# xiezhy6/PASTA-GAN

Measured on AMD Instinct MI355X. Metric: training images/sec at 256x192 (tensor 256x256), batch 16 per GPU, higher is better.
Workload: dtype f32

## Files before the change

### pasta-gan_amd/csrc/conv_igemm.hip

```cpp
#include "conv_launch.h"

namespace pasta {

static void launch_fwd_bf16x6(bool tile128, bool rows, const ConvFwdParams& p, hipStream_t s) {
    const int BM = tile128 ? 128 : 64, BN = tile128 ? 128 : 256;
    ConvFwdParams q = p;
    q.o_tiles = (p.Og + BM - 1) / BM;
    int64_t tiles = 0;
    for (int c = 0; c < p.ncls; c++) {
        const int64_t t = ceil_div64((int64_t)p.N * p.cls[c].P * p.cls[c].Q, BN);
        if (t > tiles) tiles = t;
    }
    tiles *= p.ncls;
    const dim3 grid((unsigned)tiles, q.o_tiles * q.ksplit, p.G);
    if (rows) { if (tile128) tu_fwd_rows_128(q, grid, s); else tu_fwd_rows_64(q, grid, s); }
    else      { if (tile128) tu_fwd_base_128(q, grid, s); else tu_fwd_base_64(q, grid, s); }
}

static void launch_fwd_rows2d(int kernel, const ConvFwdParams& p, hipStream_t s) {
    ConvFwdParams q = p;
    q.rows_y0 = p.tap_dy[0];
    for (int t = 1; t < 9; t++) q.rows_y0 = p.tap_dy[t] < q.rows_y0 ? p.tap_dy[t] : q.rows_y0;
    if (kernel == PASTA_FWD_ROWS2D_WIDE) { if (q.x_pieces) tu_rows2d_wide_pieces(q, s); else tu_rows2d_wide(q, s); }
    else if (kernel == PASTA_FWD_ROWS2D_R4) tu_rows2d_128_r4(q, s);
    else if (kernel == PASTA_FWD_ROWS2D_R2) tu_rows2d_128_r2(q, s);
    else tu_rows2d_64_r8(q, s);
}

static void launch_lattice(const FwdChoice& c, const ConvFwdParams& p, hipStream_t s) {
    if (c.kernel == PASTA_FWD_F32) tu_fwd_f32(c.tile, p, s);
    else if (is_rows2d(c.kernel)) launch_fwd_rows2d(c.kernel, p, s);
    else launch_fwd_bf16x6(c.tile == T128x128, c.kernel == PASTA_FWD_ROWS, p, s);
}

static void set_lattice(ConvFwdParams& p, const TapTable& t) {
    p.ncls = t.ncls;
    for (int c = 0; c < 4; c++) p.cls[c] = {t.cls[c].P, t.cls[c].Q, t.cls[c].oy0, t.cls[c].ox0, t.cls[c].T, t.cls[c].tap0};
    memcpy(p.tap_dy, t.tap_dy, sizeof(p.tap_dy)); memcpy(p.tap_dx, t.tap_dx, sizeof(p.tap_dx)); memcpy(p.tap_slab, t.tap_slab, sizeof(p.tap_slab));
    p.isy = t.isy; p.isx = t.isx; p.osy = t.osy; p.osx = t.osx;
    p.rows = t.rows; p.rows_d0 = t.rows_d0; p.rows_rev = t.rows_rev;
    const TapTable::Lattice& l = t.cls[t.ncls > 0 ? t.ncls - 1 : 0];
    p.P = l.P; p.Q = l.Q; p.oy0 = l.oy0; p.ox0 = l.ox0; p.T = l.T;
}

static float desc_wscale(const pasta_conv_desc* d) { return d->wscale == 0.f ? 1.f : d->wscale; }

static inline int launch_flags_of(const float* iscale, const float* oscale, const pasta_conv_epilogue* ep, const float* wmod_s) {
    return (iscale ? PASTA_PLAN_ISCALE : 0) | (oscale ? PASTA_PLAN_OSCALE : 0) | (ep ? PASTA_PLAN_EPILOGUE : 0) | (wmod_s ? PASTA_PLAN_MODULATED : 0) |
           (ep && ep->noise ? PASTA_PLAN_NOISE : 0);
}

static void launch_transposed_pairs(const pasta_conv_desc* d, const ConvFwdParams& base, FwdTile tile, hipStream_t s, const EdgeWeights& ew) {
    TapTable rem;
    lattice_pair_remainder(d, rem);
    if (rem.ncls) {
        ConvFwdParams q = base;
        set_lattice(q, rem);
        tu_conv_t2_edge(q, ew, s);
    }
    PairLattice pl;
    lattice_pair_main(d, pl);
    ConvFwdParams p = base;
    set_lattice(p, pl.t);
    p.pair_bx = pl.pair_bx;
    for (int i = 0; i < 3; i++) p.pair_off[i] = pl.pair_off[i];
    if (tile == T128x128) tu_fwd_pair_128(p, s); else tu_fwd_pair_64(p, s);
}

static int conv2d_run(const void* x, const float* w, void* y, const float* iscale, const float* oscale,
                      const pasta_conv_epilogue* ep, const pasta_conv_desc* d, void* workspace, int64_t workspace_bytes,
                      void* stream, const float* wmod_s, const float* wmod_d);
static int wgrad_run(const void* xv, const void* dyv, float* dw, const pasta_conv_desc* d, void* workspace, int64_t workspace_bytes, void* stream,
                     const float* mod_s, const float* mod_w, float* ds);

static bool pack_job_of(const pasta_conv_desc* d, void* workspace, PackJob& j) {
    const FwdChoice c = choose_fwd(d, 0);
    FwdWorkspace lay;
    if (c.pieces != NP_F16X3 || c.packed || d->io_dtype != PASTA_F32 || d->x2 || fwd_workspace(d, c.plan, lay)) return false;
    const int Ig = d->C_in / d->groups, Og = d->C_out / d->groups;
    j.rowinv = (float*)workspace + lay.rowinv;
    j.wp = (float*)workspace + lay.pack;
    j.G = d->groups; j.Ig = Ig; j.Og = Og;
    j.Ig_pad = round_up(Ig, fwd_ipad(Ig, c.tile)); j.Og_pad = round_up(Og, fwd_tile_bm(c.tile));
    j.kh = d->kh; j.kw = d->kw; j.transposed = d->transposed; j.flip = d->flip;
    j.wscale = desc_wscale(d);
    j.pack_xcd_rows = (j.Og_pad & 63) == 0 ? 1 : 0;
    return true;
}

}


extern "C" int64_t pasta_conv2d_workspace(const pasta_conv_desc* d) {
    using namespace pasta;
    FwdWorkspace lay;
    if (check_desc(d, "conv2d_workspace") || fwd_workspace(d, plan_fwd(d), lay)) return -1;
    return lay.total_floats * (int64_t)sizeof(float);
}

extern "C" int pasta_conv2d_tile(const pasta_conv_desc* d) {
    using namespace pasta;
    if (check_desc(d, "conv2d_tile")) return -1;
    return (int)plan_fwd(d).tile;
}

extern "C" int pasta_conv2d_plan(const pasta_conv_desc* d, int launch_flags, int* tile, int* ksplit, int* math, int* launches, int* kernel) {
    using namespace pasta;
    if (int e = check_desc(d, "conv2d_plan")) return e;
    const FwdChoice c = choose_fwd(d, launch_flags);
    if (d->io_dtype != PASTA_F32 && !c.pieces && !is_fewch(c.kernel))
        return fail("conv2d: no 16-bit-storage kernel for this shape (fewer than 16 input channels per group, at most 32 "
                    "output channels, or an input scale -- pointwise layers over more than 8192 pixels excepted): convert the tensors to fp32 for this launch");
    if (tile) *tile = (int)c.tile;
    if (ksplit) *ksplit = c.ksplit;
    if (math) *math = c.math;
    if (launches) *launches = c.launches;
    if (kernel) *kernel = c.kernel;
    if (d->x_layout == PASTA_LAYOUT_PIECES16 && !c.pieces_ok)
        return fail("conv2d: x_layout = PASTA_LAYOUT_PIECES16 is served by the 3x3 stride-2 forward kernel (conv2d, pad 0, fp32 y, PASTA_MATH_F16X3, one group, "
                    "C_in a multiple of 8 and >= 16, C_out > 32, output width a power of two >= 16, more than 8192 output pixels, no scale vectors) and by the "
                    "eight-wave 3x3 stride-1 tile kernel (plan kernel 7, no input scale, C_in a multiple of 8) only");
    return 0;
}

extern "C" int pasta_conv2d(const void* x, const float* w, void* y, const float* iscale, const float* oscale,
                            const pasta_conv_desc* d, void* workspace, int64_t workspace_bytes, void* stream) {
    return pasta_conv2d_ex(x, w, y, iscale, oscale, nullptr, d, workspace, workspace_bytes, stream);
}

extern "C" int pasta_conv2d_ex(const void* x, const float* w, void* y, const float* iscale, const float* oscale,
                               const pasta_conv_epilogue* ep, const pasta_conv_desc* d, void* workspace, int64_t workspace_bytes,
                               void* stream) {
    return pasta::conv2d_run(x, w, y, iscale, oscale, ep, d, workspace, workspace_bytes, stream, nullptr, nullptr);
}

extern "C" int pasta_conv2d_modulated(const void* x, const float* w, const float* styles, const float* dcoefs, void* y,
                                      const pasta_conv_epilogue* ep, const pasta_conv_desc* d, void* workspace, int64_t workspace_bytes,
                                      void* stream) {
    using namespace pasta;
    PASTA_CHECK(styles, "conv2d_modulated: null styles");
    return conv2d_run(x, w, y, nullptr, nullptr, ep, d, workspace, workspace_bytes, stream, styles, dcoefs);
}

extern "C" int pasta_conv2d_pack_pair(const float* w, const pasta_conv_desc* da, void* ws_a, int64_t ws_a_bytes, const pasta_conv_desc* db, void* ws_b,
                                      int64_t ws_b_bytes, void* stream, int* packed_mask) {
    using namespace pasta;
    PASTA_CHECK(w && da && db && ws_a && ws_b && packed_mask, "conv2d_pack_pair: null pointer");
    *packed_mask = 0;
    if (int e = check_desc(da, "conv2d_pack_pair")) return e;
    if (int e = check_desc(db, "conv2d_pack_pair")) return e;
    PASTA_CHECK(ws_a_bytes >= pasta_conv2d_workspace(da) && ws_b_bytes >= pasta_conv2d_workspace(db), "conv2d_pack_pair: workspace too small");
    PASTA_CHECK((((uintptr_t)ws_a | (uintptr_t)ws_b) & 15) == 0, "conv2d_pack_pair: workspaces must be 16-byte aligned");
    PackJob a, b;
    if (da->groups != db->groups || !pack_job_of(da, ws_a, a) || !pack_job_of(db, ws_b, b)) return 0;
    tu_pack_weights_f16x3_pair(w, a, b, (hipStream_t)stream);
    *packed_mask = 3;
    return launch_status("conv2d_pack_pair");
}

int pasta::conv2d_run(const void* x, const float* w, void* y, const float* iscale, const float* oscale,
                      const pasta_conv_epilogue* ep, const pasta_conv_desc* d, void* workspace, int64_t workspace_bytes,
                      void* stream, const float* wmod_s, const float* wmod_d) {
    if (int e = check_desc(d, "conv2d")) return e;
    PASTA_CHECK(!ep || (ep->act >= 1 && ep->act <= 3), "conv2d: fused epilogue supports act 1..3 (linear, relu, lrelu), got %d", ep ? ep->act : 0);
    PASTA_CHECK(!ep || !ep->noise || ep->noise_strength, "conv2d: noise without noise_strength");
    PASTA_CHECK(x && w && y, "conv2d: null pointer");
    const FwdChoice ch = choose_fwd(d, launch_flags_of(iscale, oscale, ep, wmod_s));
    FwdWorkspace lay;
    if (int e = fwd_workspace(d, ch.plan, lay)) return e;
    const int64_t need = lay.total_floats * (int64_t)sizeof(float);
    PASTA_CHECK(workspace && workspace_bytes >= need, "conv2d: workspace of %lld bytes needed, %lld given", (long long)need, (long long)workspace_bytes);
    PASTA_CHECK(((uintptr_t)workspace & 15) == 0, "conv2d: workspace must be 16-byte aligned");
    hipStream_t s = (hipStream_t)stream;
    if (is_fewch(ch.kernel)) {
        FewChParams q;
        q.x = x; q.w = w; q.y = y; q.iscale = iscale; q.io = d->io_dtype;
        q.bias = ep ? ep->bias : nullptr; q.res = ep ? ep->res : nullptr; q.y_amax = ep ? ep->y_amax : nullptr;
        q.N = d->N; q.Cin = d->C_in; q.Cout = d->C_out; q.HW = d->H * d->W;
        q.w_io = d->transposed ? 1 : 0;
        q.wscale = desc_wscale(d);
        q.act = ep ? ep->act : 0; q.alpha = ep ? ep->alpha : 0.f; q.gain = ep ? ep->gain : 1.f; q.clamp = ep ? ep->clamp : -1.f;
        tu_conv1x1_fewch(ch.kernel == PASTA_FWD_FEWCIN ? 1 : 2, q, s);
        return launch_status("conv2d");
// ... 259 lines not shown
```

### pasta-gan_amd/csrc/conv_launch.h

```cpp
#pragma once
#include "conv_common.h"

namespace pasta {

void tu_pack_weights_f32(const float* w, float* wp, int G, int Ig, int Og, int Ig_pad, int Og_pad, int kh, int kw, int transposed, int flip,
                         float wscale, const float* mod_s, const float* mod_d, hipStream_t s);
void tu_pack_weights_bf16(const float* w, void* wp, int G, int Ig, int Og, int Ig_pad, int Og_pad, int kh, int kw, int transposed, int flip,
                          float wscale, int f16, const float* mod_s, const float* mod_d, hipStream_t s);
void tu_pack_weights_f16x3(const float* w, void* wp, float* rowinv, int G, int Ig, int Og, int Ig_pad, int Og_pad, int kh, int kw, int transposed,
                           int flip, float wscale, const float* mod_s, const float* mod_d, int pack_xcd_rows, hipStream_t s);
void tu_pack_weights_f16x3_pair(const float* w, const PackJob& a, const PackJob& b, hipStream_t s);
void tu_fwd_f32(FwdTile t, const ConvFwdParams& p, hipStream_t s);

void tu_fwd_base_128(const ConvFwdParams& q, dim3 grid, hipStream_t s);
void tu_fwd_base_64(const ConvFwdParams& q, dim3 grid, hipStream_t s);
void tu_fwd_rows_128(const ConvFwdParams& q, dim3 grid, hipStream_t s);
void tu_fwd_rows_64(const ConvFwdParams& q, dim3 grid, hipStream_t s);
void tu_fwd_pair_128(const ConvFwdParams& p, hipStream_t s);
void tu_fwd_pair_64(const ConvFwdParams& p, hipStream_t s);

void tu_rows2d_wide(const ConvFwdParams& q, hipStream_t s);
void tu_rows2d_wide_pieces(const ConvFwdParams& q, hipStream_t s);
void tu_rows2d_128_r4(const ConvFwdParams& q, hipStream_t s);
void tu_rows2d_128_r2(const ConvFwdParams& q, hipStream_t s);
void tu_rows2d_64_r8(const ConvFwdParams& q, hipStream_t s);

void tu_conv1x1(const ConvFwdParams& p, hipStream_t s);
void tu_conv3x3s2(const ConvFwdParams& p, hipStream_t s);

void tu_conv_t2(const ConvFwdParams& p, hipStream_t s);

void tu_conv1x1_fewch(int kind, const FewChParams& p, hipStream_t s);

void tu_splitk_reduce(const ConvFwdParams& p, hipStream_t s);
void tu_amax_times(const float* parts_in, const float* v, int n, float* parts_out, hipStream_t s);
struct EdgeWeights { const float* w; const float* mod_s; const float* mod_d; float wscale; int flip; };
void tu_conv_t2_edge(const ConvFwdParams& q, const EdgeWeights& ew, hipStream_t s);
void tu_packed_koff(unsigned* koff, int K, int kh, int kw, int flip, int HWp, int Wp, hipStream_t s);
void tu_pad_planes(const float* x, float* xp, int64_t planes, int H, int W, int ph, int pw, hipStream_t s);

int  tu_wgrad_f32(int TR, int TS, int WA, int pipe, int kp, const WgradParams& p, int64_t blocks, size_t lds_bytes, hipStream_t s);
void tu_wgrad_reduce(const float* slab, float* dw, int ksplit, int G, int Ag, int Bg, int Ag_pad, int Bg_pad, int kh, int kw, int flip, float wscale,
                     hipStream_t s);
void tu_wgrad_reduce_modulated(bool mod_a, dim3 grid, const float* slab, const float* sty, const float* w, float* dw, float* dsp, int ksplit, int N,
                               int Ag, int Bg, int Ap, int Bp, int kh, int kw, int flip, float wscale, int wg_rows, hipStream_t s);
void tu_sum_blocks(const float* blocks, float* out, int nblocks, int n, hipStream_t s);
void tu_wgrad_smallcin(const WgradSmallParams& q, int blocks, size_t lds_bytes, hipStream_t s);
void tu_wgrad_smallcin_reduce(const float* slab, float* dw, int ksplit, int Ag, int bprime, int a_pad, int bpad, float wscale, hipStream_t s);
void tu_wgrad1x1_fewcin(int CI, int io, dim3 grid, const void* dy, const void* x, float* slab, int N, int Co, int HW, int64_t quads_per_slice, int a_pad,
                        int bpad, hipStream_t s);

void tu_wgrad3x3(int np, const WgradParams& p, int64_t blocks, hipStream_t s);
void tu_wgrad3x3s2(int np, const WgradParams& p, int64_t blocks, hipStream_t s);
void tu_wgrad1x1(int np, int WA, const WgradParams& p, int64_t blocks, hipStream_t s);

}
```

### pasta-gan_amd/csrc/conv_plan.h

```cpp
#ifndef PASTA_CONV_PLAN_H
#define PASTA_CONV_PLAN_H
#include <stddef.h>
#include <stdlib.h>
#include "../../include/pasta_hip.h"
#include "host_common.h"

namespace pasta {

constexpr int MAX_TAPS = 49;
constexpr int NP_F16X3 = 4;
constexpr int AMAX_PARTS = 256;
constexpr int WS_AMAX_FLOATS = 2 * AMAX_PARTS;

enum FwdTile { T128x128 = 0, T64x256 = 1, T32x256 = 2, T64x64 = 3 };

static inline int fwd_tile_bm(FwdTile t) { return t == T128x128 ? 128 : t == T32x256 ? 32 : 64; }
static inline int fwd_tile_bn(FwdTile t) { return t == T128x128 ? 128 : 256; }

static inline int round_up(int a, int b) { return (a + b - 1) / b * b; }


static inline bool is_rows2d(int k) { return k >= PASTA_FWD_ROWS2D_R4 && k <= PASTA_FWD_ROWS2D_WIDE; }
static inline bool is_fewch(int k) { return k == PASTA_FWD_FEWCIN || k == PASTA_FWD_FEWCOUT; }
static inline bool wgrad_split(int k) { return k == PASTA_WGRAD_3X3 || k == PASTA_WGRAD_3X3S2 || k == PASTA_WGRAD_1X1 || k == PASTA_WGRAD_3X3S2_PIECES; }


static inline int check_desc(const pasta_conv_desc* d, const char* who) {
    PASTA_CHECK(d, "%s: null descriptor", who);
    PASTA_CHECK(d->N >= 1 && d->C_in >= 1 && d->H >= 1 && d->W >= 1 && d->C_out >= 1 && d->OH >= 1 && d->OW >= 1,
                "%s: empty tensor in descriptor", who);
    PASTA_CHECK(d->kh >= 1 && d->kw >= 1 && d->kh * d->kw <= MAX_TAPS, "%s: kernel %dx%d unsupported (max %d taps)", who, d->kh, d->kw, MAX_TAPS);
    PASTA_CHECK(d->stride >= 1 && d->stride <= 4, "%s: stride %d unsupported", who, d->stride);
    PASTA_CHECK(d->pad_h >= 0 && d->pad_w >= 0, "%s: negative padding", who);
    PASTA_CHECK(d->math >= PASTA_MATH_DEFAULT && d->math <= PASTA_MATH_F16X3, "%s: unknown math mode %d", who, d->math);
    PASTA_CHECK(d->io_dtype == PASTA_F32 || d->io_dtype == PASTA_F16 || d->io_dtype == PASTA_BF16, "%s: io_dtype %d is not PASTA_F32 / PASTA_F16 / PASTA_BF16", who, d->io_dtype);
    PASTA_CHECK(d->groups >= 1 && d->C_in % d->groups == 0 && d->C_out % d->groups == 0, "%s: channels not divisible by groups=%d", who, d->groups);
    PASTA_CHECK(d->x_layout == PASTA_LAYOUT_NCHW || d->x_layout == PASTA_LAYOUT_PIECES16, "%s: unknown x_layout %d", who, d->x_layout);
    if (!d->transposed) {
        const int oh = (d->H + 2 * d->pad_h - d->kh) / d->stride + 1, ow = (d->W + 2 * d->pad_w - d->kw) / d->stride + 1;
        PASTA_CHECK(d->H + 2 * d->pad_h >= d->kh && d->W + 2 * d->pad_w >= d->kw && oh == d->OH && ow == d->OW,
                    "%s: conv2d output is %dx%d, descriptor says %dx%d", who, oh, ow, d->OH, d->OW);
    } else {
        const int oh = (d->H - 1) * d->stride - 2 * d->pad_h + d->kh, ow = (d->W - 1) * d->stride - 2 * d->pad_w + d->kw;
        PASTA_CHECK(d->OH >= oh && d->OH < oh + d->stride && d->OW >= ow && d->OW < ow + d->stride,
                    "%s: conv_transpose2d output %dx%d not in [%d,%d)x[%d,%d)", who, d->OH, d->OW, oh, oh + d->stride, ow, ow + d->stride);
    }
    PASTA_CHECK((int64_t)d->N * d->C_in * d->H * d->W <= INT32_MAX && (int64_t)d->N * d->C_out * d->OH * d->OW <= INT32_MAX,
                "%s: tensor too large", who);
    return 0;
}


static inline bool split_arith(const pasta_conv_desc* d) { return d->math != PASTA_MATH_F32 || d->io_dtype != PASTA_F32; }
static inline bool doubled_plane(const pasta_conv_desc* d) { return d->OH >= 2 * d->H && d->OH <= 2 * d->H + 1 && d->OW >= 2 * d->W && d->OW <= 2 * d->W + 1; }
static inline bool doubled_remainder(const pasta_conv_desc* d) { return d->OH > 2 * d->H || d->OW > 2 * d->W; }
static inline bool is_3x3(const pasta_conv_desc* d) { return d->kh == 3 && d->kw == 3; }
static inline bool pads_0_or_1(const pasta_conv_desc* d) { return d->pad_h == d->pad_w && d->pad_h <= 1; }

struct SLDims { int P, Q, LH, LW; };
static inline SLDims sl_dims(const pasta_conv_desc* d) {
    return d->transposed ? SLDims{d->H, d->W, d->OH, d->OW} : SLDims{d->OH, d->OW, d->H, d->W};
}

static inline int math_pieces(int math) { return math == PASTA_MATH_BF16 ? 1 : math == PASTA_MATH_BF16X3 ? 2 : math == PASTA_MATH_BF16X6 ? 3 : NP_F16X3; }
static inline bool fp32_equivalent(int pieces) { return pieces == 3 || pieces == NP_F16X3; }


static inline bool rows_tile_ok(int P, int Q, int BN) {
    const int seg = Q < BN ? Q : BN;
    return Q % 32 == 0 && (seg & (seg - 1)) == 0 && BN % seg == 0 && Q % seg == 0 && ((int64_t)P * Q) % BN == 0;
}

template <int BN, int R>
static inline bool rows2d_tile_ok(int P, int Q) {
    constexpr int SEG = BN / R;
    return P % R == 0 && Q % SEG == 0;
}
static inline int rows2d_rows(int P, int Q) {
    if (rows2d_tile_ok<128, 4>(P, Q)) return 4;
    return rows2d_tile_ok<128, 2>(P, Q) ? 2 : 0;
}
static inline bool rows2d_r8(int P, int Q) { return rows2d_tile_ok<256, 8>(P, Q); }

static inline bool conv3x3s2_shape_ok(int OH, int OW) {
    if (OW < 16 || (OW & (OW - 1))) return false;
    const int seg = OW < 128 ? OW : 128, R = 128 / seg;
    return OH % R == 0;
}

static inline int conv1x1_fewch_kind(const pasta_conv_desc* d, bool has_iscale, bool has_oscale, bool has_noise, bool modulated) {
    if (d->kh != 1 || d->kw != 1 || d->stride != 1 || d->pad_h || d->pad_w || d->groups != 1) return 0;
    if (has_oscale || has_noise || modulated || d->x2 || d->x_layout || d->OH != d->H || d->OW != d->W) return 0;
    const int64_t hw = (int64_t)d->H * d->W;
    if (hw % 4 || (int64_t)d->N * hw <= 8192) return 0;
    if (d->C_in <= 16 && !has_iscale && d->C_out >= 16 && d->C_out <= 512) return 1;
    if (d->C_out <= 16 && d->C_in >= 16 && (int64_t)d->C_in * ((d->C_out + 3) & ~3) * 4 <= 64 * 1024) return 2;
    return 0;
}

static inline int wgrad_mod_rows(int Ap, int Bp, int KK) { return (int64_t)(Bp / 64) * (Ap / 16) * KK >= 512 ? 16 : 4; }

struct WgradChunks { int cw_log2, qblocks, chunks_total; };
static inline WgradChunks wgrad_chunks(int kp, int rows_total, int Q, bool keep_width = false) {
    WgradChunks c;
    int cw = kp, lg = kp == 32 ? 5 : 4;
    while (cw > 1 && cw / 2 >= Q && !keep_width) { cw /= 2; lg--; }
    const int chh = kp / cw;
    c.cw_log2 = lg;
    c.qblocks = (Q + cw - 1) / cw;
    c.chunks_total = ((rows_total + chh - 1) / chh) * c.qblocks;
    return c;
}


static inline int fwd_ipad(int Ig, FwdTile t) { return (Ig <= 4 && t == T64x256) ? 4 : Ig <= 8 ? 8 : 16; }

static inline int64_t fwd_lattice_pixels(const pasta_conv_desc* d) {
    if (!d->transposed) return (int64_t)d->N * d->OH * d->OW;
    return (int64_t)d->N * ((d->OH + d->stride - 1) / d->stride) * ((d->OW + d->stride - 1) / d->stride);
}

struct FwdPlan { FwdTile tile; int ksplit; int bf16x6; int packed; };

static inline bool isc_in_staging(const pasta_conv_desc* d) { return d->io_dtype == PASTA_F32 && fp32_equivalent(math_pieces(d->math)); }

static inline FwdPlan plan_fwd(const pasta_conv_desc* d) {
    const int Og = d->C_out / d->groups, Ig = d->C_in / d->groups;
    const int64_t npix = fwd_lattice_pixels(d);
    const bool sb = split_arith(d) && Ig >= 16 && (int64_t)d->N * d->C_in * d->H * d->W < (1ll << 30);
    const bool few = !d->transposed && d->groups == 1 && Ig < 16 && Og > 32 && npix > 8192 && d->io_dtype == PASTA_F32 &&
                     d->math != PASTA_MATH_F32 && fp32_equivalent(math_pieces(d->math)) && Ig * d->kh * d->kw >= 64 && Ig * d->kh * d->kw <= 1024 &&
                     (int64_t)d->N * d->C_in * (d->H + 2 * d->pad_h) * (d->W + 2 * d->pad_w) < (1ll << 28);
    FwdPlan f;
    f.packed = few;
    if (Og <= 32 && !(sb && Og > 16 && npix > 8192)) f.tile = T32x256;
    else if (npix <= 8192) f.tile = (sb && Og > 64) ? T128x128 : T64x64;
    else if (Og <= 64) f.tile = T64x256;
    else f.tile = T128x128;
    f.bf16x6 = (sb || few) && (f.tile == T128x128 || f.tile == T64x256);
    f.packed = f.packed && f.bf16x6;
    f.ksplit = 1;
    if (npix <= 8192 && f.tile != T32x256) {
        const int bm = fwd_tile_bm(f.tile), bn = f.tile == T64x64 ? 64 : 128;
        int64_t blocks = ceil_div64(npix, bn) * ((Og + bm - 1) / bm) * d->groups;
        const int taps = d->transposed ? 1 : d->kh * d->kw;
        if (d->transposed && f.bf16x6 && d->stride == 2) blocks *= 4;
        const int64_t k_total = (int64_t)taps * round_up(Ig, 16);
        int64_t ks = (f.tile == T64x64 ? 768 : 512) / (blocks > 0 ? blocks : 1);
        if (ks > k_total / 64) ks = k_total / 64;
        if (ks > 32) ks = 32;
        f.ksplit = ks < 2 ? 1 : (int)ks;
    }
    return f;
}

static inline bool merged_classes(const pasta_conv_desc* d, bool bf16x6) {
    return d->transposed && bf16x6 && d->stride == 2 && d->OH >= 2 && d->OW >= 2;
}

static inline bool t2_3x3_doubled(const pasta_conv_desc* d, int ksplit) {
    return d->transposed && d->stride == 2 && is_3x3(d) && d->io_dtype == PASTA_F32 && ksplit == 1 && doubled_plane(d);
}

static inline bool pair_launch_ok(const pasta_conv_desc* d, int pieces, int ksplit, FwdTile tile, bool pair_small) {
    if (!t2_3x3_doubled(d, ksplit) || !pads_0_or_1(d) || !fp32_equivalent(pieces)) return false;
    if (tile != T128x128 && tile != T64x256) return false;
    if (doubled_remainder(d) && (int64_t)d->H * d->W < 128 * 128 && !pair_small) return false;
    return rows_tile_ok(d->H, d->W, fwd_tile_bn(tile));
}

static inline bool t2_shape_ok(const pasta_conv_desc* d, int pieces, int ksplit) {
    if (!t2_3x3_doubled(d, ksplit) || d->pad_h != 0 || d->pad_w != 0) return false;
    if (pieces != NP_F16X3 || d->x2 || d->x_layout) return false;
    return d->C_in / d->groups >= 16 && ((d->H % 8 == 0 && d->W % 32 == 0) || (d->H % 16 == 0 && d->W % 16 == 0));
}

enum TransposedLaunch { TL_NONE, TL_ONEPASS, TL_PAIR, TL_MERGED, TL_PER_CLASS };

struct FwdChoice {
    int kernel;
    FwdPlan plan;
    FwdTile tile;
    int ksplit;
    int pieces;
    int math;
    int launches;
    TransposedLaunch tl;
    bool packed;
    bool pieces_ok;
};

static inline FwdChoice choose_fwd(const pasta_conv_desc* d, int launch_flags) {
    static const int rows2d_mode = getenv("PASTA_ROWS2D") ? atoi(getenv("PASTA_ROWS2D")) : 8;
    static const bool pair_small = getenv("PASTA_T2_PAIR") && getenv("PASTA_T2_PAIR")[0] == '2';
    const bool iscale = launch_flags & PASTA_PLAN_ISCALE, oscale = launch_flags & PASTA_PLAN_OSCALE;
    const bool modulated = launch_flags & PASTA_PLAN_MODULATED, noise = launch_flags & PASTA_PLAN_NOISE;
    const FwdPlan f = plan_fwd(d);
    const int np = math_pieces(d->math);
    const bool f32 = d->io_dtype == PASTA_F32;
    FwdChoice c;
    c.plan = f;
    c.tile = f.tile;
    c.tl = TL_NONE;
    c.packed = false;
    c.pieces = 0;
    c.pieces_ok = false;
    if (const int few = conv1x1_fewch_kind(d, iscale, oscale, noise, modulated)) {
        c.kernel = few == 1 ? PASTA_FWD_FEWCIN : PASTA_FWD_FEWCOUT; c.ksplit = 1; c.math = PASTA_MATH_F32; c.launches = 1;
        return c;
    }
    c.ksplit = f.ksplit;
    const bool sb = f.bf16x6 && (!iscale || isc_in_staging(d)) && !(f.packed && (iscale || modulated));
    c.packed = sb && f.packed;
    c.pieces = !sb ? 0 : !f32 ? 1 : np;
    c.math = !sb ? PASTA_MATH_F32 : !f32 ? PASTA_MATH_BF16 : d->math == PASTA_MATH_BF16X3 ? PASTA_MATH_BF16X3 : d->math == PASTA_MATH_BF16 ? PASTA_MATH_BF16 :
             d->math == PASTA_MATH_BF16X6 ? PASTA_MATH_BF16X6 : PASTA_MATH_F16X3;
    const bool f16x3 = sb && f32 && np == NP_F16X3;
    const int bn1 = (d->C_out / d->groups) <= 64 ? 256 : 128;
    const bool c1x1 = f16x3 && d->groups == 1 && d->kh == 1 && d->kw == 1 && d->stride == 1 && !d->pad_h && !d->pad_w && !iscale && !oscale && !noise &&
                      c.ksplit == 1 && !c.packed && d->C_in >= 16 && d->C_out > 32 && d->OH == d->H && d->OW == d->W && ((int64_t)d->H * d->W) % bn1 == 0;
    const bool s2_fits = f16x3 && !d->transposed && d->groups == 1 && is_3x3(d) && d->stride == 2 && pads_0_or_1(d) &&
                         !iscale && !oscale && c.ksplit == 1 && !c.packed && d->C_in >= 16 && d->C_out > 32 && conv3x3s2_shape_ok(d->OH, d->OW);
    const bool s2 = s2_fits && !noise;
    const bool t2 = sb && t2_shape_ok(d, np, c.ksplit) && !(launch_flags & ~(PASTA_PLAN_ISCALE | PASTA_PLAN_MODULATED));
    const bool pair = !t2 && sb && !(launch_flags & ~PASTA_PLAN_MODULATED) && pair_launch_ok(d, np, c.ksplit, c.tile, pair_small);
    const bool rows = sb && d->stride == 1 && d->kw == 3 && rows_tile_ok(d->OH, d->OW, fwd_tile_bn(c.tile));
    const bool plain6 = sb && d->stride == 1 && is_3x3(d) && rows2d_mode != 0;
    const int rows2d = plain6 && c.tile == T128x128 ? rows2d_rows(d->OH, d->OW) : 0;
    const bool rows2d_256 = plain6 && c.tile == T64x256 && rows2d_r8(d->OH, d->OW);
    const bool wide = rows2d && rows2d_mode == 8 && (!iscale || np == NP_F16X3) && fp32_equivalent(np) && f32 && rows2d_r8(d->OH, d->OW);
    c.kernel = !sb ? PASTA_FWD_F32 : c1x1 ? PASTA_FWD_1X1 : s2 ? PASTA_FWD_3X3S2 : c.packed ? PASTA_FWD_PACKED_K : t2 ? PASTA_FWD_T2 : pair ? PASTA_FWD_PAIR :
               wide ? PASTA_FWD_ROWS2D_WIDE : rows2d ? (rows2d == 4 ? PASTA_FWD_ROWS2D_R4 : PASTA_FWD_ROWS2D_R2) : rows2d_256 ? PASTA_FWD_ROWS2D_R8 :
               rows ? PASTA_FWD_ROWS : PASTA_FWD_BASE;
    if (d->transposed)
        c.tl = t2 ? TL_ONEPASS : pair ? TL_PAIR : merged_classes(d, sb) ? TL_MERGED : TL_PER_CLASS;
    c.launches = c.tl == TL_PAIR ? 1 + (doubled_remainder(d) ? 1 : 0) : c.tl != TL_PER_CLASS ? 1 :
                 (d->stride < d->OH ? d->stride : d->OH) * (d->stride < d->OW ? d->stride : d->OW);
    c.pieces_ok = f16x3 && d->groups == 1 && !(launch_flags & (PASTA_PLAN_ISCALE | PASTA_PLAN_MODULATED)) && d->C_in >= 16 && (d->C_in & 7) == 0 && !d->x2 &&
                  (wide || (s2_fits && d->pad_h == 0));
    return c;
}

struct FwdWorkspace { int64_t rowinv, pack, partial, koff, extra, total_floats; };

static inline int fwd_workspace(const pasta_conv_desc* d, const FwdPlan& f, FwdWorkspace& ws) {
    const int Ig = d->C_in / d->groups, Og_pad = round_up(d->C_out / d->groups, fwd_tile_bm(f.tile));
    int64_t pack = ((int64_t)d->groups * d->kh * d->kw * round_up(Ig, fwd_ipad(Ig, f.tile)) * Og_pad * 3 + 1) / 2;
    const int64_t partial = f.ksplit > 1 ? (int64_t)f.ksplit * d->N * d->C_out * d->OH * d->OW : 0;
    int64_t koff = 0, extra = 0;
    if (f.packed) {
        koff = round_up(Ig * d->kh * d->kw, 16);
        const int64_t pk = (koff * Og_pad * 3 + 1) / 2;
        pack = pack > pk ? pack : pk;
        if (d->pad_h || d->pad_w) extra = (int64_t)d->N * d->C_in * (d->H + 2 * d->pad_h) * (d->W + 2 * d->pad_w);
    }
    const bool t2 = t2_shape_ok(d, math_pieces(d->math), f.ksplit);
    if (t2) { koff = 0; extra = (int64_t)d->N * d->C_in * d->H; }
    PASTA_CHECK(!(f.packed || t2) || partial == 0, "conv2d: the packed-K table and the one-pass kernel's column exist without K slices only");
    ws.rowinv = WS_AMAX_FLOATS;
    ws.pack = ws.rowinv + (int64_t)d->groups * Og_pad;
    ws.partial = ws.pack + round_up((int)pack, 4);
    ws.koff = ws.partial + partial;
    ws.extra = ws.koff + koff;
    ws.total_floats = ws.koff + round_up((int)(koff + extra), 4);
    return 0;
}


struct WgradPlan {
    int TR, TS, WA, WB, pipe, npos, kp, bf16x6, tgr, tgs, a_tiles, b_tiles, cw_log2, qblocks, chunks_total, ksplit, rows_total;
    int64_t slab_floats; size_t lds_bytes;
};

static inline bool wgrad_3x3s1_same(const pasta_conv_desc* d, const SLDims& t) {
    return split_arith(d) && is_3x3(d) && d->stride == 1 && d->pad_h == 1 && d->pad_w == 1 && t.LH == t.P && t.LW == t.Q;
}

static inline bool wgrad_wide16(const pasta_conv_desc* d) {
    const SLDims t = sl_dims(d);
    return wgrad_3x3s1_same(d, t) && t.Q == 16 && !d->x_layout;
}

static inline WgradPlan plan_wgrad(int N, int P, int Q, int G, int Ag, int Bg, int kh, int kw, int st, int ks_multiple = 1, bool wide16 = false) {
    WgradPlan w;
    w.bf16x6 = 0;
    if (kh == 3 && kw == 3) { w.TR = 3; w.TS = 3; }
    else if (kw == 7) { w.TR = 1; w.TS = 7; }
    else if (kw == 4) { w.TR = 1; w.TS = 4; }
    else { w.TR = 1; w.TS = 1; }
    w.WA = w.WB = (w.TR * w.TS == 1 && Ag > 64 && Bg > 64) ? 2 : 1;
    const int BA = 64 * w.WA, BB = 64 * w.WB;
    w.tgr = (kh + w.TR - 1) / w.TR; w.tgs = (kw + w.TS - 1) / w.TS;
    w.a_tiles = (Ag + BA - 1) / BA; w.b_tiles = (Bg + BB - 1) / BB;
    int kp = 32;
    w.rows_total = N * P;
    for (;;) {
        const WgradChunks c = wgrad_chunks(kp, w.rows_total, Q, wide16);
        const int cw = 1 << c.cw_log2, chh = kp >> c.cw_log2;
        const int lwid = (cw - 1) * st + w.TS;
        w.cw_log2 = c.cw_log2; w.qblocks = c.qblocks; w.chunks_total = c.chunks_total;
        w.kp = kp; w.npos = chh * w.TR * lwid;
        if (w.npos <= 128 || kp == 16) break;
        kp = 16;
    }
    const int cw = 1 << w.cw_log2, chh = w.kp >> w.cw_log2;
    const int64_t base_blocks = (int64_t)G * w.a_tiles * w.b_tiles * w.tgr * w.tgs;
    int64_t ks = (512 + base_blocks / 2) / base_blocks;
    if (ks > w.chunks_total / 8) ks = w.chunks_total / 8;
    if (ks < 1) ks = 1;
    if (ks > 1024) ks = 1024;
    if (ks_multiple > 1) ks = (ks + ks_multiple - 1) / ks_multiple * ks_multiple;
    w.ksplit = (int)ks;
    w.slab_floats = (int64_t)w.ksplit * G * kh * kw * w.a_tiles * BA * w.b_tiles * BB;
    const int lwid = (cw - 1) * st + w.TS, lpitch = lwid | 1, lch = (chh * w.TR * lpitch) | 1;
    w.lds_bytes = (size_t)(BA * (w.kp + 1) + BB * lch) * sizeof(float);
    w.pipe = w.npos <= 128 ? 1 : 0;
    return w;
}

struct WgradSmallPlan { bool use; int nb, bprime, cw_log2, qblocks, chunks_total, ksplit, a_tiles, rows_total; int64_t slab_floats; size_t lds_bytes; };

static inline WgradSmallPlan plan_wgrad_small(const pasta_conv_desc* d) {
    WgradSmallPlan w{}; w.use = false;
    const int Ig = d->C_in / d->groups;
    if (d->transposed || d->groups != 1 || d->stride != 1 || d->flip || Ig > 8 || Ig * d->kh * d->kw > 160) return w;
    w.use = true;
    w.bprime = Ig * d->kh * d->kw; w.nb = (w.bprime + 31) / 32;
    w.rows_total = d->N * d->OH;
    const WgradChunks c = wgrad_chunks(32, w.rows_total, d->OW);
    w.cw_log2 = c.cw_log2; w.qblocks = c.qblocks; w.chunks_total = c.chunks_total;
    const int cw = 1 << c.cw_log2, chh = 32 >> c.cw_log2;
    w.a_tiles = (d->C_out + 63) / 64;
    int64_t ks = (1024 + w.a_tiles - 1) / w.a_tiles;
    if (ks > w.chunks_total / 8) ks = w.chunks_total / 8;
    if (ks < 1) ks = 1;
    w.ksplit = (int)ks;
    w.slab_floats = (int64_t)w.ksplit * w.a_tiles * 64 * w.nb * 32;
    w.lds_bytes = (size_t)(64 * 33 + Ig * chh * d->kh * (cw + d->kw - 1) + 4) * sizeof(float);
    if (Ig * chh * d->kh * (cw + d->kw - 1) > 1024) w.use = false;
    return w;
}

static inline int plan_wgrad1x1_fewcin(const pasta_conv_desc* d, const WgradSmallPlan& ws) {
    if (!ws.use || d->kh != 1 || d->kw != 1 || d->pad_h || d->pad_w || d->C_in > 8) return 0;
    const int64_t hw = (int64_t)d->H * d->W;
    if (hw % 4 || d->OH != d->H || d->OW != d->W) return 0;
    int64_t ks = (int64_t)d->N * (hw / 4) / (256 * 8);
    ks = ks < 1 ? 1 : ks > 256 ? 256 : ks;
    return (int)(ks < ws.ksplit ? ks : ws.ksplit);
}

static inline bool wgrad_bf16x6(const pasta_conv_desc* d, const WgradPlan& w) {
    const SLDims t = sl_dims(d);
    return wgrad_3x3s1_same(d, t) && (t.Q % 32 == 0 || wgrad_wide16(d)) && w.kp == 32 && w.cw_log2 == 5;
}
static inline bool wgrad_s2_bf16x6(const pasta_conv_desc* d, const WgradPlan& w) {
    return split_arith(d) && is_3x3(d) && d->stride == 2 && pads_0_or_1(d) && sl_dims(d).Q % 16 == 0 && w.kp == 16 && w.cw_log2 == 4;
}
static inline bool wgrad_pieces_ok(const pasta_conv_desc* d, const WgradPlan& w) {
    return d->x_layout == PASTA_LAYOUT_PIECES16 && wgrad_s2_bf16x6(d, w) && !d->transposed && d->pad_h == 0 && d->groups == 1 && d->io_dtype == PASTA_F32 &&
           math_pieces(d->math) == NP_F16X3 && (d->C_in & 7) == 0;
}
static inline bool wgrad_1x1_bf16x6(const pasta_conv_desc* d, const WgradPlan& w) {
    const SLDims t = sl_dims(d);
    const int Ig = d->C_in / d->groups, Og = d->C_out / d->groups;
    return split_arith(d) && d->kh == 1 && d->kw == 1 && d->stride == 1 && d->pad_h == 0 && d->pad_w == 0 &&
           ((int64_t)t.P * t.Q) % 32 == 0 && (Ig >= 16 || Og >= 16) && w.kp == 32 && w.WA == w.WB &&
           d->H == d->OH && d->W == d->OW && (int64_t)w.chunks_total == (int64_t)d->N * t.P * t.Q / 32;
}

// ... 161 lines not shown
```

Measured before the change: 122.0.

## Add whole-plane 3x3 forward conv kernel for 8x8 and 16x16 feature maps

```diff
diff --git a/pasta-gan_amd/csrc/conv_fwd_planes.h b/pasta-gan_amd/csrc/conv_fwd_planes.h
--- /dev/null
+++ b/pasta-gan_amd/csrc/conv_fwd_planes.h
@@ -0,0 +1,240 @@
+#pragma once
+#include "conv_common.h"
+
+namespace pasta {
+
+template <int BM, int BN, int PL, bool ISC, int NT>
+__global__ __launch_bounds__(NT, NT == 256 ? 2 : 1) void conv_fwd_planes_f16x3_kernel(ConvFwdParams p) {
+    constexpr int NP = NP_F16X3, IO = IO_F32;
+    constexpr int NPA = Arith<NP>::npa, NPB = Arith<NP>::npb;
+    constexpr unsigned ES = io_size<IO>::value;
+    constexpr int WMT = 2, WNT = 2, KC = 16;
+    constexpr int WAVES_N = BN / 64;
+    static_assert((BM / 64) * WAVES_N == NT / 64, "one wave per 64 x 64 sub-tile");
+    constexpr int PP = PL * PL, IMGS = BN / PP, SW = PL + 2, ISL = SW * SW, SLOTS = IMGS * ISL;
+    static_assert(IMGS * PP == BN, "whole planes fill the pixel tile");
+    constexpr int UNITS = 2 * SLOTS, UPT = (UNITS + NT - 1) / NT;
+    static_assert(UPT <= 3, "at most three staging units per thread and chunk");
+    constexpr int USTRIDE = 3;
+    constexpr int AUNITS = 2 * NPA * BM, APT = (AUNITS + NT - 1) / NT;
+    constexpr int ABUF = APT * NT * 8, BSEG = SLOTS * 8, BBUF = 2 * NPB * BSEG;
+    extern __shared__ __attribute__((aligned(16))) __bf16 planes_smem[];
+    __bf16* const As = planes_smem;
+    __bf16* const Bs = planes_smem + 2 * ABUF;
+
+    const int tid = threadIdx.x, lane = tid & 63, wave = __builtin_amdgcn_readfirstlane(tid >> 6);
+    const int wm = wave / WAVES_N, wn = wave % WAVES_N;
+    const int g = blockIdx.z;
+    const int ks = blockIdx.y / p.o_tiles;
+    const int o_blk = (blockIdx.y - ks * p.o_tiles) * BM;
+    const int HW = p.H * p.W;
+    const int NC = p.Ig_pad / KC;
+    const int c_first = (int)(((unsigned)NC * (unsigned)ks) / (unsigned)p.ksplit);
+    const int nchunks = (int)(((unsigned)NC * (unsigned)(ks + 1)) / (unsigned)p.ksplit) - c_first;
+    const int n0 = blockIdx.x * IMGS;
+    const int ymin = p.rows_y0, d0 = p.rows_d0;
+
+    const char* const xbytes = (const char*)p.x;
+    const __bf16* wb = (const __bf16*)p.wp + (int64_t)g * p.KK * NC * 6 * p.Og_pad * 8;
+    const int64_t a_chunk = (int64_t)6 * p.Og_pad * 8;
+
+    unsigned u_pix[UPT];
+    bool u_ok[UPT];
+    int u_half[UPT], u_lds[UPT], u_isc[ISC ? UPT : 1];
+#pragma unroll
+    for (int k = 0; k < UPT; k++) {
+        const int u = tid + NT * k;
+        const int half = u >= SLOTS ? 1 : 0;
+        int slot = u - half * SLOTS;
+        const bool real = u < UNITS;
+        slot = real ? slot : 0;
+        const int img = slot / ISL, rem = slot - img * ISL;
+        const int i = rem / SW, j = rem - i * SW;
+        const int y = ymin + i, x = d0 + j, n = n0 + img;
+        u_ok[k] = real && n < p.N && (unsigned)y < (unsigned)p.H && (unsigned)x < (unsigned)p.W;
+        const int nn = u_ok[k] ? n : n0;
+        const int chan0 = nn * p.Cin + g * p.Ig;
+        u_pix[k] = (unsigned)chan0 * (unsigned)HW * ES + (u_ok[k] ? (unsigned)(y * p.W + x) * ES : 0u);
+        if constexpr (ISC) u_isc[k] = chan0;
+        u_half[k] = half;
+        u_lds[k] = real ? (half * SLOTS + slot) * 8 : -1;
+    }
+
+    float sb0[8], sb1[8];
+    float sc0[ISC ? 8 : 1], sc1[ISC ? 8 : 1];
+    int nv0 = 0, nv1 = 0;
+    auto load_unit = [&](int k, int cc, bool real_chunk, float (&sb)[8], float (&sc)[ISC ? 8 : 1], int& nv) {
+        const int c0 = cc * KC + u_half[k] * 8;
+        const int last = p.Ig - 1;
+#pragma unroll
+        for (int j = 0; j < 8; j++) {
+            const int c = c0 + j < last ? c0 + j : last;
+            sb[j] = io_ld<IO>(xbytes, u_pix[k] + (unsigned)c * (unsigned)HW * ES);
+            if constexpr (ISC) sc[j] = p.iscale[u_isc[k] + c];
+        }
+        nv = (u_ok[k] && real_chunk) ? p.Ig - c0 : 0;
+    };
+    const __bf16* wtap[9];
+#pragma unroll
+    for (int t = 0; t < 9; t++) wtap[t] = wb + (int64_t)p.tap_slab[t] * NC * a_chunk;
+    float4 areg0, areg1, areg2, breg0, breg1, breg2;
+    auto load_a = [&](int tap, int cc, int set) {
+        const int ccl = cc < NC ? cc : NC - 1;
+        const __bf16* wt = wtap[tap] + (int64_t)ccl * a_chunk;
+        auto unit = [&](int j) {
+            int e = tid + NT * j;
+            if (NT * (j + 1) > AUNITS) e = e < AUNITS ? e : AUNITS - 1;
+            const int seg = e / BM, within = e - seg * BM;
+            return *(const float4*)(wt + ((int64_t)seg * p.Og_pad + o_blk + within) * 8);
+        };
+        if (set == 0) { areg0 = unit(0); if (APT > 1) areg1 = unit(1); if (APT > 2) areg2 = unit(2); }
+        else          { breg0 = unit(0); if (APT > 1) breg1 = unit(1); if (APT > 2) breg2 = unit(2); }
+    };
+    load_a(0, c_first, 0);
+    float fb[UPT][8], fc[UPT][ISC ? 8 : 1];
+    int fnv[UPT];
+#pragma unroll
+    for (int k = 0; k < UPT; k++) load_unit(k, c_first < NC ? c_first : NC - 1, nchunks > 0, fb[k], fc[k], fnv[k]);
+
+    float x_scale, out_scale;
+    scale_from_amax(amax_of_parts(p.x_amax), x_scale, out_scale);
+    uint32_t q1[4], q2[4];
+    auto split_pair = [&](const float (&sb)[8], const float (&sc)[ISC ? 8 : 1], int nv, int j) {
+        float v0 = sb[2 * j], v1 = sb[2 * j + 1];
+        if constexpr (ISC) { v0 *= sc[2 * j]; v1 *= sc[2 * j + 1]; }
+        if (nv < 8) {
+            v0 = 2 * j < nv ? v0 : 0.f;
+            v1 = 2 * j + 1 < nv ? v1 : 0.f;
+        }
+        f16_split2(v0 * x_scale, v1 * x_scale, q1[j], q2[j]);
+    };
+    auto store_unit = [&](int k, int bbuf) {
+        if (u_lds[k] >= 0) {
+            __bf16* bd = Bs + bbuf * BBUF + u_lds[k];
+            *(uint4*)(bd) = make_uint4(q1[0], q1[1], q1[2], q1[3]);
+            *(uint4*)(bd + 2 * BSEG) = make_uint4(q2[0], q2[1], q2[2], q2[3]);
+        }
+    };
+    auto store_a = [&](int buf, int set) {
+        __bf16* d = As + buf * ABUF;
+        *(float4*)&d[tid * 8] = set ? breg0 : areg0;
+        if (APT > 1) *(float4*)&d[(tid + NT) * 8] = set ? breg1 : areg1;
+        if (APT > 2) *(float4*)&d[(tid + 2 * NT) * 8] = set ? breg2 : areg2;
+    };
+
+    f32x16 acc[WMT][WNT];
+#pragma unroll
+    for (int a = 0; a < WMT; a++)
+#pragma unroll
+        for (int b = 0; b < WNT; b++)
+#pragma unroll
+            for (int r = 0; r < 16; r++) acc[a][b][r] = 0.f;
+
+    const int hl = lane >> 5, jl = lane & 31;
+    uint32_t y_am = 0;
+    const AmaxSlot y_slot = amax_begin(p.y_amax);
+    int fslot[WNT];
+#pragma unroll
+    for (int b = 0; b < WNT; b++) {
+        const int t = (wn * WNT + b) * 32 + jl;
+        const int img = t / PP, rem = t - img * PP;
+        const int r = rem / PL, c = rem - r * PL;
+        fslot[b] = img * ISL + r * SW + c;
+    }
+    int toff[9];
+#pragma unroll
+    for (int t = 0; t < 9; t++) toff[t] = (p.tap_dy[t] - ymin) * SW + (p.tap_dx[t] - d0);
+
+    struct Frag { bf16x8_t a[WMT][3], b[WNT][2]; };
+    auto read_frag = [&](Frag& f, int abuf, int bbuf, int off) {
+        const __bf16* A_ = As + abuf * ABUF;
+        const __bf16* B_ = Bs + bbuf * BBUF;
+#define PASTA_LDA(PC) { _Pragma("unroll") for (int a = 0; a < WMT; a++) f.a[a][PC] = *(const bf16x8_t*)&A_[(((PC) * 2 + hl) * BM + (wm * WMT + a) * 32 + jl) * 8]; }
+#define PASTA_LDB(PC) { _Pragma("unroll") for (int b = 0; b < WNT; b++) f.b[b][PC] = *(const bf16x8_t*)&B_[(((PC) * 2 + hl) * SLOTS + fslot[b] + off) * 8]; }
+        PASTA_LDA(2) PASTA_LDB(1) PASTA_LDA(1) PASTA_LDB(0) PASTA_LDA(0)
+#undef PASTA_LDA
+#undef PASTA_LDB
+    };
+
+    auto step = [&](const int S, const int PAR, int cc) {
+        const int gpar = (PAR * 9 + S) & 1;
+        const bool next_real = cc + 1 < c_first + nchunks;
+        constexpr int NOUNIT = -1;
+        int ku = NOUNIT;
+#pragma unroll
+        for (int k = 0; k < UPT; k++)
+            if (S == (USTRIDE * (k + 1) < 8 ? USTRIDE * (k + 1) : 8)) ku = k;
+        if (S + 2 < 9) load_a(S + 2, cc, gpar); else load_a(S + 2 - 9, cc + 1, gpar);
+#pragma unroll
+        for (int k = 0; k < UPT; k++)
+            if (S == USTRIDE * k) {
+                if ((k & 1) == 0) load_unit(k, next_real ? cc + 1 : cc, next_real, sb0, sc0, nv0);
+                else              load_unit(k, next_real ? cc + 1 : cc, next_real, sb1, sc1, nv1);
+            }
+        Frag f;
+        read_frag(f, gpar, PAR, toff[S]);
+#define PASTA_MM(PA, PB)                                                                                         \
+        _Pragma("unroll") for (int a = 0; a < WMT; a++) _Pragma("unroll") for (int b = 0; b < WNT; b++)          \
+            acc[a][b] = mfma16<IO, NP>(f.a[a][PA], f.b[b][PB], acc[a][b]);
+#define PASTA_SPLIT(J) if (ku != NOUNIT) { if ((ku & 1) == 0) split_pair(sb0, sc0, nv0, J); else split_pair(sb1, sc1, nv1, J); }
+        PASTA_MM(2, 1)
+        PASTA_SPLIT(0)
+        PASTA_SPLIT(1)
+        PASTA_MM(1, 0)
+        PASTA_SPLIT(2)
+        PASTA_SPLIT(3)
+        if (ku != NOUNIT) store_unit(ku, PAR ^ 1);
+        store_a(gpar ^ 1, gpar ^ 1);
+        PASTA_MM(0, 0)
+#undef PASTA_MM
+#undef PASTA_SPLIT
+        __syncthreads();
+    };
+
+#pragma unroll
+    for (int k = 0; k < UPT; k++) {
+#pragma unroll
+        for (int j = 0; j < 4; j++) split_pair(fb[k], fc[k], fnv[k], j);
+        store_unit(k, 0);
+    }
+    store_a(0, 0);
+    load_a(1, c_first, 1);
+    __syncthreads();
+    for (int c = 0; c < nchunks; c += 2) {
+        const int cc = c_first + c;
+        step(0, 0, cc); step(1, 0, cc); step(2, 0, cc); step(3, 0, cc); step(4, 0, cc); step(5, 0, cc); step(6, 0, cc); step(7, 0, cc); step(8, 0, cc);
+        step(0, 1, cc + 1); step(1, 1, cc + 1); step(2, 1, cc + 1); step(3, 1, cc + 1); step(4, 1, cc + 1); step(5, 1, cc + 1); step(6, 1, cc + 1); step(7, 1, cc + 1); step(8, 1, cc + 1);
+    }
+
+    conv_unscale_rows<WMT, WNT>(p.w_rowinv + (int64_t)g * p.Og_pad + o_blk, out_scale, wm, lane, acc);
+    const float nstr = (p.noise && p.ksplit == 1) ? p.noise_strength[0] : 0.f;
+    const EpiAct ea = conv_epi_act(p.act, p.alpha, p.gain, p.clamp, p.ksplit == 1);
+    conv_epilogue_dispatch<true>(o_blk + BM <= p.Og, ea, [&](auto full_c, auto case_c) {
+#pragma unroll
+        for (int b = 0; b < WNT; b++) {
+            const int t = (wn * WNT + b) * 32 + jl;
+            const int img = t / PP, rem = t - img * PP;
+            const int r = rem / PL, c = rem - r * PL;
+            const int n = n0 + img;
+            if (n >= p.N) continue;
+            const EpiColumn col = conv_epi_column(p, ea, g, ks, n, r * p.OW + c, nstr);
+#pragma unroll
+            for (int a = 0; a < WMT; a++)
+                conv_store_subtile<IO>(acc[a][b], col, o_blk + (wm * WMT + a) * 32, p.Og, lane, ea, y_am, full_c, case_c);
+        }
+    });
+    if (p.ksplit == 1) amax_commit(y_am, y_slot);
+}
+
+template <int PL, bool ISC>
+static void launch_fwd_planes(const ConvFwdParams& q, hipStream_t s) {
+    constexpr int BM = 128, BN = 256, NT = 512;
+    constexpr int SLOTS = (BN / (PL * PL)) * (PL + 2) * (PL + 2);
+    constexpr int APT = (2 * Arith<NP_F16X3>::npa * BM + NT - 1) / NT;
+    constexpr size_t lds = (size_t)(2 * APT * NT * 8 + 2 * 2 * Arith<NP_F16X3>::npb * SLOTS * 8) * sizeof(__bf16);
+    const dim3 grid((unsigned)((q.N + BN / (PL * PL) - 1) / (BN / (PL * PL))), q.o_tiles * q.ksplit, q.G);
+    PASTA_SET_LDS((conv_fwd_planes_f16x3_kernel<BM, BN, PL, ISC, NT>), lds);
+    hipLaunchKernelGGL((conv_fwd_planes_f16x3_kernel<BM, BN, PL, ISC, NT>), grid, dim3(NT), lds, s, q);
+}
+
+}
diff --git a/pasta-gan_amd/csrc/conv_igemm.hip b/pasta-gan_amd/csrc/conv_igemm.hip
--- a/pasta-gan_amd/csrc/conv_igemm.hip
+++ b/pasta-gan_amd/csrc/conv_igemm.hip
@@ -28,7 +28,8 @@
 }
 
 static void launch_lattice(const FwdChoice& c, const ConvFwdParams& p, hipStream_t s) {
-    if (c.kernel == PASTA_FWD_F32) tu_fwd_f32(c.tile, p, s);
+    if (c.planes) tu_fwd_planes(c.planes, p, s);
+    else if (c.kernel == PASTA_FWD_F32) tu_fwd_f32(c.tile, p, s);
     else if (is_rows2d(c.kernel)) launch_fwd_rows2d(c.kernel, p, s);
     else launch_fwd_bf16x6(c.tile == T128x128, c.kernel == PASTA_FWD_ROWS, p, s);
 }
diff --git a/pasta-gan_amd/csrc/conv_launch.h b/pasta-gan_amd/csrc/conv_launch.h
--- a/pasta-gan_amd/csrc/conv_launch.h
+++ b/pasta-gan_amd/csrc/conv_launch.h
@@ -24,6 +24,8 @@
 void tu_rows2d_128_r4(const ConvFwdParams& q, hipStream_t s);
 void tu_rows2d_128_r2(const ConvFwdParams& q, hipStream_t s);
 void tu_rows2d_64_r8(const ConvFwdParams& q, hipStream_t s);
+
+void tu_fwd_planes(int side, const ConvFwdParams& p, hipStream_t s);
 
 void tu_conv1x1(const ConvFwdParams& p, hipStream_t s);
 void tu_conv3x3s2(const ConvFwdParams& p, hipStream_t s);
diff --git a/pasta-gan_amd/csrc/conv_plan.h b/pasta-gan_amd/csrc/conv_plan.h
--- a/pasta-gan_amd/csrc/conv_plan.h
+++ b/pasta-gan_amd/csrc/conv_plan.h
@@ -120,8 +120,21 @@
     return (int64_t)d->N * ((d->OH + d->stride - 1) / d->stride) * ((d->OW + d->stride - 1) / d->stride);
 }
 
-struct FwdPlan { FwdTile tile; int ksplit; int bf16x6; int packed; };
-
+struct FwdPlan { FwdTile tile; int ksplit; int bf16x6; int packed; int planes; };
+
+constexpr int PLANES_BN = 256;
+static inline int fwd_planes_blocks(const pasta_conv_desc* d, int side) {
+    const int imgs = PLANES_BN / (side * side);
+    return ((d->N + imgs - 1) / imgs) * ((d->C_out / d->groups + 127) / 128) * d->groups;
+}
+static inline int fwd_planes(const pasta_conv_desc* d) {
+    if (!is_3x3(d) || d->stride != 1 || d->pad_h != 1 || d->pad_w != 1 || d->H != d->W || d->OH != d->H || d->OW != d->W) return 0;
+    if (d->H != 8 && d->H != 16) return 0;
+    if (d->io_dtype != PASTA_F32 || math_pieces(d->math) != NP_F16X3 || d->x2 || d->x_layout) return 0;
+    if (d->C_in / d->groups < 16 || d->C_out / d->groups <= 64 || (int64_t)d->N * d->C_in * d->H * d->W >= (1ll << 30)) return 0;
+    if (fwd_planes_blocks(d, d->H) < 16) return 0;
+    return d->H;
+}
 static inline bool isc_in_staging(const pasta_conv_desc* d) { return d->io_dtype == PASTA_F32 && fp32_equivalent(math_pieces(d->math)); }
 
 static inline FwdPlan plan_fwd(const pasta_conv_desc* d) {
@@ -140,6 +153,7 @@
     f.bf16x6 = (sb || few) && (f.tile == T128x128 || f.tile == T64x256);
     f.packed = f.packed && f.bf16x6;
     f.ksplit = 1;
+    f.planes = (sb && !few && f.tile == T128x128) ? fwd_planes(d) : 0;
     if (npix <= 8192 && f.tile != T32x256) {
         const int bm = fwd_tile_bm(f.tile), bn = f.tile == T64x64 ? 64 : 128;
         int64_t blocks = ceil_div64(npix, bn) * ((Og + bm - 1) / bm) * d->groups;
@@ -151,6 +165,10 @@
         if (ks > 32) ks = 32;
         f.ksplit = ks < 2 ? 1 : (int)ks;
     }
+    if (f.planes) {
+        const int nc = round_up(Ig, 16) / 16;
+        if (2 * f.ksplit > nc) f.ksplit = nc / 2 < 2 ? 1 : nc / 2;
+    }
     return f;
 }
 
@@ -187,6 +205,7 @@
     int launches;
     TransposedLaunch tl;
     bool packed;
+    int planes;
     bool pieces_ok;
 };
 
@@ -203,6 +222,7 @@
     c.tile = f.tile;
     c.tl = TL_NONE;
     c.packed = false;
+    c.planes = 0;
     c.pieces = 0;
     c.pieces_ok = false;
     if (const int few = conv1x1_fewch_kind(d, iscale, oscale, noise, modulated)) {
@@ -216,6 +236,7 @@
     c.math = !sb ? PASTA_MATH_F32 : !f32 ? PASTA_MATH_BF16 : d->math == PASTA_MATH_BF16X3 ? PASTA_MATH_BF16X3 : d->math == PASTA_MATH_BF16 ? PASTA_MATH_BF16 :
              d->math == PASTA_MATH_BF16X6 ? PASTA_MATH_BF16X6 : PASTA_MATH_F16X3;
     const bool f16x3 = sb && f32 && np == NP_F16X3;
+    c.planes = f16x3 ? f.planes : 0;
     const int bn1 = (d->C_out / d->groups) <= 64 ? 256 : 128;
     const bool c1x1 = f16x3 && d->groups == 1 && d->kh == 1 && d->kw == 1 && d->stride == 1 && !d->pad_h && !d->pad_w && !iscale && !oscale && !noise &&
                       c.ksplit == 1 && !c.packed && d->C_in >= 16 && d->C_out > 32 && d->OH == d->H && d->OW == d->W && ((int64_t)d->H * d->W) % bn1 == 0;
diff --git a/pasta-gan_amd/csrc/conv_tu_fwd_planes.hip b/pasta-gan_amd/csrc/conv_tu_fwd_planes.hip
--- /dev/null
+++ b/pasta-gan_amd/csrc/conv_tu_fwd_planes.hip
@@ -0,0 +1,13 @@
+#include "conv_launch.h"
+#include "conv_fwd_planes.h"
+
+namespace pasta {
+void tu_fwd_planes(int side, const ConvFwdParams& p, hipStream_t s) {
+    ConvFwdParams q = p;
+    q.o_tiles = (p.Og + 127) / 128;
+    q.rows_y0 = p.tap_dy[0];
+    for (int t = 1; t < 9; t++) q.rows_y0 = p.tap_dy[t] < q.rows_y0 ? p.tap_dy[t] : q.rows_y0;
+    if (side == 16)     { if (q.iscale) launch_fwd_planes<16, true>(q, s); else launch_fwd_planes<16, false>(q, s); }
+    else                { if (q.iscale) launch_fwd_planes<8, true>(q, s);  else launch_fwd_planes<8, false>(q, s); }
+}
+}
```

Result: no change. 122.3, median of 6 (+0.2%).
